# maleiwhat/Our-Tree

Hardware: AMD Instinct MI355X
Metric: GB/s AES-128-CTR (whole node) (higher is better)
Workload: dtype uint8

## Files before the change

csrc/cpu/bs_selftest.cpp:

```cpp
#include <stdio.h>
#include <stdlib.h>
#include <string.h>

#include <utility>

#include "aes.h"
#include "otc_bitslice.h"

using namespace otc_bs;


template <int... G, int... Q>
static void dfs_step(W *m, int step, std::integer_sequence<int, G...>, std::integer_sequence<int, Q...>)
{
    ((step == G ? transpose32_nib8<G>(m) : (void)0), ...);
    ((step == 8 + Q ? transpose32_quad<Q>(m) : (void)0), ...);
    ((step == 16 + G ? transpose32_group8<G>(m) : (void)0), ...);
}

extern "C" int otc_bs_dfs_transpose(uint32_t *m, const int *steps, int nsteps)
{
    for (int i = 0; i < nsteps; ++i) {
        const int s = steps[i];
        if (!((s >= 0 && s < 4) || (s >= 8 && s < 16) || (s >= 16 && s < 20))) return -1;
    }
    transpose32_bytes(m);
    for (int i = 0; i < nsteps; ++i)
        dfs_step(m, steps[i], std::make_integer_sequence<int, 4>{}, std::make_integer_sequence<int, 8>{});
    return 0;
}

extern "C" int otc_bs_ctr_out_model(const uint32_t *planes, const uint32_t *rk, const uint32_t *pt, uint32_t *out,
                                    int dfs, int ls, int first, int cap, int *order)
{
    W s[128];
    for (int p = 0; p < 128; ++p) s[p] = planes[p];
    int issued[32], emitted[32], nemit = 0, err = 0;
    uint32_t reg[32][4];
    for (int k = 0; k < 32; ++k) {
        issued[k] = k < first;
        emitted[k] = 0;
        for (int w = 0; w < 4; ++w) reg[k][w] = issued[k] ? pt[4 * k + w] : 0xDEADBEEFu;
        if (order) order[k] = -1;
    }
    auto emit = [&](int k) {
        if (!issued[k]) err = err ? err : 1;
        if (emitted[k]++) err = err ? err : 2;
        for (int w = 0; w < 4; ++w) out[4 * k + w] = x3(reg[k][w], s[32 * w + k], rk[w]);
        ++nemit;
    };
    auto issue = [&](int j) {
        if (j < first || issued[j]++) err = err ? err : 2;
        for (int w = 0; w < 4; ++w) reg[j][w] = pt[4 * j + w];
        if (order) order[j] = nemit;
    };
    if (!dfs) {
        for (int w = 0; w < 4; ++w) transpose32(s + 32 * w);
        for (int j = first; j < 32; ++j) issue(j);
        for (int k = 0; k < 32; ++k) emit(k);
    } else if (ls == 8 && first == 10 && cap == 36) {
        ctr_out_dfs<8, 10, 36>(s, emit, issue);
    } else if (ls == 8 && first == 10 && cap == 34) {
        ctr_out_dfs<8, 10, 34>(s, emit, issue);
    } else if (ls == 12 && first == 14 && cap == 36) {
        ctr_out_dfs<12, 14, 36>(s, emit, issue);
    } else if (ls == 0 && first == 4 && cap == 40) {
        ctr_out_dfs<0, 4, 40>(s, emit, issue);
    } else {
        return -1;
    }
    for (int k = 0; k < 32; ++k)
        if (!issued[k] || emitted[k] != 1) err = err ? err : 2;
    return err;
}

extern "C" int otc_bitslice_selftest(int verbose)
{
    const uint8_t *SB = aes_sbox();
    int fails = 0;
    for (int batch = 0; batch < 8; ++batch) {
        W x[8] = {0};
        for (int k = 0; k < 32; ++k) {
            int v = batch * 32 + k;
            for (int i = 0; i < 8; ++i) x[i] |= (W)((v >> i) & 1) << k;
        }
        sbox(x[0], x[1], x[2], x[3], x[4], x[5], x[6], x[7]);
        for (int k = 0; k < 32; ++k) {
            int v = batch * 32 + k, o = 0;
            for (int i = 0; i < 8; ++i) o |= (int)((x[i] >> k) & 1) << i;
            if (o != SB[v]) {
                if (verbose) printf("  sbox mismatch at %02x: %02x vs %02x\n", v, o, SB[v]);
                ++fails;
            }
        }
    }
    for (int kv = 0; kv < 256; kv += 37) {
        W k[8], x[8] = {0}, y[8];
        for (int i = 0; i < 8; ++i) k[i] = ((kv >> i) & 1) ? ~0u : 0u;
        for (int slot = 0; slot < 32; ++slot)
            for (int i = 0; i < 8; ++i) x[i] |= (W)(((slot * 7 + kv) >> i) & 1) << slot;
        for (int i = 0; i < 8; ++i) y[i] = x[i] ^ k[i];
        sbox(y[0], y[1], y[2], y[3], y[4], y[5], y[6], y[7]);
        W z[8];
        for (int i = 0; i < 8; ++i) z[i] = x[i];
        sbox_k<false>(x[0], x[1], x[2], x[3], x[4], x[5], x[6], x[7], k[0], k[1], k[2], k[3], k[4], k[5], k[6], k[7]);
        sbox_lut3(z[0], z[1], z[2], z[3], z[4], z[5], z[6], z[7], k[0], k[1], k[2], k[3], k[4], k[5], k[6], k[7]);
        for (int i = 0; i < 8; ++i)
            if (x[i] != y[i] || z[i] != y[i]) {
                if (verbose) printf("  sbox_k/sbox_lut3 mismatch kv=%d bit %d\n", kv, i);
                ++fails;
            }
    }
    for (int t = 0; t < 64; ++t) {
        W a[32], b[32];
        uint64_t z = 0x9E3779B97F4A7C15ull * (uint64_t)(t + 1);
        for (int i = 0; i < 32; ++i) {
            z ^= z << 13; z ^= z >> 7; z ^= z << 17;
            a[i] = b[i] = (W)(z >> 11);
        }
        W c[32];
        for (int i = 0; i < 32; ++i) c[i] = a[i];
        transpose32(a);
        transpose32_ref(b);
        for (int i = 0; i < 32; ++i)
            if (a[i] != b[i]) {
                if (verbose) printf("  transpose32 mismatch (trial %d, word %d)\n", t, i);
                ++fails;
                break;
// ... 81 lines not shown
                else round_step<0>(s, kr);
            }
            round_final(s, [&](int p) -> W { return kf(ctx.nr - 1, p); });
            bad = 0;
            for (int w = 0; w < 4; ++w) {
                W m[32];
                for (int q = 0; q < 32; ++q) m[q] = s[32 * w + q];
                transpose32(m);
                for (int k = 0; k < 32; ++k) {
                    uint32_t v = m[k] ^ rk[4 * ctx.nr + w];
                    bad += memcmp(&v, &ref[k][4 * w], 4) != 0;
                }
            }
            if (verbose)
                printf("  bitsliced AES-%d rolled rounds%s: %s\n", bits,
                       mixt == 2 ? " (searched 55-node MixColumns)" : mixt ? " (low-register MixColumns)" : "",
                       bad ? "failed" : "passed");
            fails += bad;
        }

        {
            static uint32_t tab[14 * 16 * OTC_BS_KT_STRIDE];
            key_term_table(rk, ctx.nr, tab);
            for (int w = 0; w < 4; ++w) {
                W m[32];
                for (int k = 0; k < 32; ++k) memcpy(&m[k], &pt[k][4 * w], 4);
                transpose32(m);
                for (int q = 0; q < 32; ++q) s[32 * w + q] = m[q];
            }
            for (int r = 0; r + 1 < ctx.nr; ++r)
                round_step_kt<true>(s, [&](int b, W *t) {
                    for (int j = 0; j < OTC_SBOX_KEY_TERMS; ++j) t[j] = tab[(r * 16 + b) * OTC_BS_KT_STRIDE + j];
                });
            round_final_kt(s, [&](int b, W *t) {
                for (int j = 0; j < OTC_SBOX_KEY_TERMS; ++j) t[j] = tab[((ctx.nr - 1) * 16 + b) * OTC_BS_KT_STRIDE + j];
            });
            bad = 0;
            for (int w = 0; w < 4; ++w) {
                W m[32];
                for (int q = 0; q < 32; ++q) m[q] = s[32 * w + q];
                transpose32(m);
                for (int k = 0; k < 32; ++k) {
                    uint32_t v = m[k] ^ rk[4 * ctx.nr + w];
                    bad += memcmp(&v, &ref[k][4 * w], 4) != 0;
                }
            }
            if (verbose) printf("  bitsliced AES-%d key-term table rounds: %s\n", bits, bad ? "failed" : "passed");
            fails += bad;

            bad = 0;
            for (int trial = 0; trial < 4; ++trial) {
                uint64_t hi = ((uint64_t)rand() << 32) ^ (uint64_t)rand();
                uint64_t lo = (((uint64_t)rand() << 32) ^ (uint64_t)rand()) & ~(uint64_t)2047u;
                if (trial == 3) lo = ~(uint64_t)0 << 11;
                const uint32_t u5 = (uint32_t)(lo >> 11) & 31u;
                uint8_t ctr[16];
                for (int b = 0; b < 8; ++b) ctr[b] = (uint8_t)(hi >> (8 * (7 - b)));
                for (int b = 0; b < 8; ++b) ctr[8 + b] = (uint8_t)(lo >> (8 * (7 - b)));
                uint8_t pre[14];
                ctr_group_prefix(lo, hi, false, 0, pre);
                bad += memcmp(pre, ctr, 14) != 0;
                static uint32_t grp[OTC_BS_CTR_GRP_WORDS];
                uint32_t c8[8], e1w[OTC_BS_CTR_E1_WORDS];
                ctr_group_consts(pre, rk, sbox_value, c8, grp);
                const uint32_t k14 = (rk[3] >> 16) & 0xFFu, k15 = rk[3] >> 24;
                ctr_e1_task(c8, k14, u5, sbox_value, e1w);
                for (int lane = 0; lane < 64; lane += 21) {
                    uint32_t ent[8];
                    ctr_e0_lane(c8, k15, (uint32_t)lane, sbox_value, ent);
                    W e0[32], e1[32];
                    for (int p = 0; p < 32; ++p) {
                        e0[p] = rep_byte(ent[p >> 2], p & 3);
                        e1[p] = e1w[p];
                    }
                    ctr_round2_mix(e0, e1, s);
                    round_step_kt<true>(s, [&](int b, W *t) {
                        for (int j = 0; j < OTC_SBOX_KEY_TERMS; ++j) t[j] = grp[b * OTC_BS_KT_STRIDE + j];
                    });
                    for (int r = 3; r + 1 < ctx.nr; ++r)
                        round_step_kt<true>(s, [&](int b, W *t) {
                            for (int j = 0; j < OTC_SBOX_KEY_TERMS; ++j) t[j] = tab[(r * 16 + b) * OTC_BS_KT_STRIDE + j];
                        });
                    round_final_kt(s, [&](int b, W *t) {
                        for (int j = 0; j < OTC_SBOX_KEY_TERMS; ++j)
                            t[j] = tab[((ctx.nr - 1) * 16 + b) * OTC_BS_KT_STRIDE + j];
                    });
                    for (int w = 0; w < 4; ++w) {
                        W m[32];
                        for (int q = 0; q < 32; ++q) m[q] = s[32 * w + q];
                        transpose32(m);
                        for (int k = 0; k < 32; ++k) {
                            uint8_t cb[16], ks[16];
                            memcpy(cb, ctr, 16);
                            const uint32_t add = 64u * (uint32_t)k + (uint32_t)lane;
                            cb[15] = (uint8_t)add;
                            cb[14] = (uint8_t)((u5 << 3) | (add >> 8));
                            aes_crypt_ecb(&ctx, AES_ENCRYPT, cb, ks);
                            uint32_t v = m[k] ^ rk[4 * ctx.nr + w];
                            bad += memcmp(&v, &ks[4 * w], 4) != 0;
                        }
                    }
                }
            }
            if (verbose) printf("  bitsliced AES-%d counter-cached CTR task: %s\n", bits, bad ? "failed" : "passed");
            fails += bad;
        }
    }
    return fails ? 1 : 0;
}
```

csrc/hip/aes_bs.hip:

```cpp
#include <hip/hip_runtime.h>

#include <cstdlib>
#include <cstring>
#include <type_traits>

#include "otc_bitslice.h"
#include "otc_device.h"
#include "otc_kernels.h"

using namespace otc_dev;
using namespace otc_bs;

namespace {

struct BsParams {
    const uint8_t *in;
    uint8_t *out;
    uint64_t nblocks;
    uint32_t tail;
    uint32_t wrap64;
    uint64_t shift;
    Ctr128 cbase;
    const uint32_t *ktab;
    const uint32_t *ctab;
// ... 73 lines not shown
        task = gw == 0 ? 0 : P.tasks - 1;
    }
    t.vbase = task * 2048u;
    if (t.vbase >= P.nblocks + shift) return false;
    t.full = t.vbase >= shift && t.vbase + 2048u - shift <= P.nblocks;
    if (P.part == BS_FULL_ONLY && !t.full) return false;
    if (P.part == BS_EDGE_ONLY && t.full) return false;
    return true;
}

#ifndef OTC_BS_NT
#define OTC_BS_NT 1
#endif
constexpr bool BS_NT = OTC_BS_NT != 0;
constexpr bool BS_NT_IN = BS_NT;
constexpr int BS_LDS_AUX = BS_NT ? 2 : 0;
__device__ __forceinline__ uint4 ld_stream(const uint8_t *p) { return ld_u4<BS_NT>(p); }
__device__ __forceinline__ void st_stream(uint8_t *p, uint4 v) { st_u4<BS_NT>(p, v); }

template <int MODE>
__device__ __forceinline__ void ecb_load_planes(const BsParams &P, const Task &t, W *s, bool full)
{
    constexpr int64_t BACK = MODE == BS_CFB_DEC ? 16 : 0;
    const uint8_t *tb = P.in + (int64_t)(t.vbase * 16) - BACK;
    const uint32_t lo = t.lane * 16u;
    uint4 blk[32];
#pragma unroll
    for (int k = 0; k < 32; ++k) {
        const uint64_t i = t.vbase + t.lane + 64u * k;
        if constexpr (MODE == BS_CFB_DEC_SEG) {
            blk[k] = seg_prev<MODE>(P, tb + lo + 1024u * k, i, full || i < P.nblocks);
        } else if (MODE == BS_CFB_DEC && k == 0) {
            const bool first = i == 0;
            const uint8_t *src = P.in + (int64_t)(t.vbase * 16) + lo - (first ? 0 : 16);
            blk[k] = blend_iv((full || i < P.nblocks) ? *(const uint4 *)src : make_uint4(0, 0, 0, 0), first, P);
        } else {
            blk[k] = (full || i < P.nblocks) ? ld_u4<BS_NT_IN>(tb + lo + 1024u * k) : make_uint4(0, 0, 0, 0);
        }
    }
#pragma unroll
    for (int w = 0; w < 4; ++w) {
        W m[32];
#pragma unroll
        for (int k = 0; k < 32; ++k) m[k] = w == 0 ? blk[k].x : w == 1 ? blk[k].y : w == 2 ? blk[k].z : blk[k].w;
        transpose32(m);
        pin_n(m, 32);
#pragma unroll
        for (int q = 0; q < 32; ++q) s[32 * w + q] = m[q];
        sched_fence();
    }
}

template <bool DEC>
__global__ __launch_bounds__(256) void k_bs_key_table(otc_aes_key K, uint32_t *tab)
{
    const int e = (int)threadIdx.x;
    if (e >= K.nr * 16) return;
    const int r = e >> 4, b = e & 15;
    uint32_t byte = (K.rk[4 * r + (b >> 2)] >> (8 * (b & 3))) & 0xFFu;
    if (DEC) byte = dec_round_key_byte(byte, r);
    W k[8];
#pragma unroll
    for (int i = 0; i < 8; ++i) k[i] = ((byte >> i) & 1u) ? ~0u : 0u;
    W t[OTC_SBOX_KEY_TERMS];
    sbox_key_terms(k[0], k[1], k[2], k[3], k[4], k[5], k[6], k[7], t);
    uint32_t *o = tab + e * OTC_BS_KT_STRIDE;
#pragma unroll
    for (int j = 0; j < OTC_SBOX_KEY_TERMS; ++j) o[j] = t[j];
    o[OTC_SBOX_KEY_TERMS] = 0;
}

using ktab_ptr = const __attribute__((address_space(4))) uint32_t *;

template <int R>
struct TableTerms {
    ktab_ptr tp;
    __device__ __forceinline__ void operator()(int b, W *t) const
    {
        ktab_ptr q = tp;
        asm volatile("" : "+s"(q));
#pragma unroll
        for (int j = 0; j < OTC_SBOX_KEY_TERMS; ++j) t[j] = q[(R * 16 + b) * OTC_BS_KT_STRIDE + j];
    }
};

template <int BASE>
struct GroupTerms {
    ktab_ptr gp;
    __device__ __forceinline__ void operator()(int b, W *t) const
    {
        ktab_ptr q = gp;
        asm volatile("" : "+s"(q));
#pragma unroll
        for (int j = 0; j < OTC_SBOX_KEY_TERMS; ++j) t[j] = q[(BASE + b) * OTC_BS_KT_STRIDE + j];
    }
};

__global__ __launch_bounds__(256) void k_bs_ctr_table(otc_aes_key K, Ctr128 cbase, uint32_t wrap64,
                                                      uint64_t ngroups, uint64_t tasks, uint32_t *gtab,
                                                      uint32_t *e0tab, uint32_t *e1tab)
{
    __shared__ uint32_t sbt[256];
    sbt[threadIdx.x] = sbox_value(threadIdx.x);
    __syncthreads();
    const auto sb = [&](uint32_t v) { return sbt[v & 0xFFu]; };
    const uint64_t i = (uint64_t)blockIdx.x * 256u + threadIdx.x;
    auto rk0b = [&](int b) -> uint32_t { return (K.rk[b >> 2] >> (8 * (b & 3))) & 0xFFu; };
    uint64_t g;
    int kind;
    if (i < ngroups) {
        g = i;
        kind = 0;
    } else if (i < ngroups * 65) {
        g = (i - ngroups) >> 6;
        kind = 1;
    } else if (i < ngroups * 65 + tasks) {
        g = (((cbase.lo >> 11) & 31u) + (i - ngroups * 65)) >> 5;
        kind = 2;
    } else {
        return;
    }
    uint8_t pre[14];
    ctr_group_prefix(cbase.lo, cbase.hi, wrap64 != 0, g, pre);
    uint32_t c8[8];
    if (kind == 0) {
        ctr_group_consts(pre, K.rk, sb, c8, gtab + g * OTC_BS_CTR_GRP_WORDS);
    } else if (kind == 1) {
        ctr_group_consts(pre, K.rk, sb, c8, (uint32_t *)nullptr);
        const uint32_t lane = (uint32_t)(i - ngroups) & 63u;
        ctr_e0_lane(c8, rk0b(15), lane, sb, e0tab + (g * 64 + lane) * 8);
    } else {
        ctr_group_consts(pre, K.rk, sb, c8, (uint32_t *)nullptr);
        const uint64_t t = i - ngroups * 65;
        const uint32_t u5 = (uint32_t)((cbase.lo >> 11) + t) & 31u;
        ctr_e1_task(c8, rk0b(14), u5, sb, e1tab + t * OTC_BS_CTR_E1_WORDS);
    }
}

template <int R, int NR, int MIX, bool DEC = false>
__device__ __forceinline__ void rounds_table(W *s, ktab_ptr tp)
{
    if constexpr (R < NR - 1) {
        round_step_kt<MIX, TableTerms<R>, 2, DEC>(s, TableTerms<R>{tp});
        pin_n(s, 128);
        rounds_table<R + 1, NR, MIX, DEC>(s, tp);
    } else {
        round_final_kt<TableTerms<NR - 1>, DEC>(s, TableTerms<NR - 1>{tp});
    }
}

#ifndef OTC_BS_CBC_D
#define OTC_BS_CBC_D 4
#endif
#ifndef OTC_BS_CFB_D
#define OTC_BS_CFB_D 2
#endif
#ifndef OTC_BS_PRE
#define OTC_BS_PRE 2
#endif
#ifndef OTC_BS_OUT_DFS
#define OTC_BS_OUT_DFS 1
#endif
#ifndef OTC_BS_DFS_CAP
#define OTC_BS_DFS_CAP 36
#endif
constexpr bool BS_OUT_DFS = OTC_BS_OUT_DFS != 0;
constexpr int BS_DFS_CAP = OTC_BS_DFS_CAP;
template <int NR, int MODE, int LS, bool CACHE, bool FO, int MIX = 2, int PRE = OTC_BS_PRE, int D = 8>
__device__ __forceinline__ void aes_bs_task(const BsParams &P, const otc_aes_key &K, uint4 *stage,
                                            int64_t claimed = -1)
{
    Task t;
    if (!task_of<MODE>(P, t, claimed)) return;
    const uint32_t lane = t.lane, wave = t.wave;
    const uint64_t shift = (MODE == BS_CTR) ? P.shift : 0;
    const bool full = FO || t.full;
    W s[128];
    auto prefetch = [&]() {
    if (MODE == BS_CTR && LS > 0) {
        const int64_t t0 = (int64_t)t.vbase - (int64_t)shift;
        const uint8_t *ib0 = P.in + t0 * 16 + lane * 16u;
#pragma unroll
        for (int k = 0; k < LS; ++k) {
            const int64_t si = t0 + (int64_t)lane + 64 * k;
            const bool ok = full || (si >= 0 && (uint64_t)si < P.nblocks);
            __builtin_amdgcn_global_load_lds((const void *)(ok ? ib0 + 1024u * k : P.in),
                                             (__attribute__((address_space(3))) void *)&stage[(wave * LS + k) * 64],
                                             16, 0, BS_LDS_AUX);
        }
    }
    };
    if (!(MODE == BS_CTR && CACHE)) prefetch();
    if (MODE == BS_CTR && CACHE) {
        const uint64_t task = t.vbase >> 11;
        const uint64_t g = (((P.cbase.lo >> 11) & 31u) + task) >> 5;
        const uint4 *q0 = (const uint4 *)(P.e0tab + (g * 64u + lane) * 8u);
        const uint4 a = q0[0], b = q0[1];
        const W ew[8] = {a.x, a.y, a.z, a.w, b.x, b.y, b.z, b.w};
        W e0[32];
#pragma unroll
        for (int p = 0; p < 32; ++p) e0[p] = rep_byte(ew[p >> 2], p & 3);
        const ktab_ptr e1p = (ktab_ptr)P.e1tab + task * OTC_BS_CTR_E1_WORDS;
        W e1[32];
#pragma unroll
        for (int p = 0; p < 32; ++p) e1[p] = e1p[p];
        const ktab_ptr gp = (ktab_ptr)P.ctab + g * OTC_BS_CTR_GRP_WORDS;
        ctr_round2_mix(e0, e1, s);
        pin_n(s, 128);
        sched_fence();
        prefetch();
        sched_fence();
        round_step_kt<MIX, GroupTerms<0>, 2>(s, GroupTerms<0>{gp});
        pin_n(s, 128);
        sched_fence();
        rounds_table<3, NR, MIX>(s, (ktab_ptr)P.ktab);
    } else if (MODE == BS_CTR) {
        const uint64_t clo = P.cbase.lo + t.vbase;
        const uint64_t chi = P.cbase.hi + ((!P.wrap64 && clo < P.cbase.lo) ? 1u : 0u);
        uint32_t cw[4] = {(uint32_t)clo, (uint32_t)(clo >> 32), (uint32_t)chi, (uint32_t)(chi >> 32)};
#pragma unroll
        for (int j = 0; j < 4; ++j) asm volatile("" : "+v"(cw[j]));
#pragma unroll
        for (int b = 0; b < 16; ++b) {
#pragma unroll
            for (int i = 0; i < 8; ++i) {
                const int n = 8 * (15 - b) + i;
                W v;
                if (n < 6) {
                    v = lane_mask(lane, n);
                } else if (n < 11) {
                    constexpr W pat[5] = {0xAAAAAAAAu, 0xCCCCCCCCu, 0xF0F0F0F0u, 0xFF00FF00u, 0xFFFF0000u};
                    v = pat[n - 6];
                } else {
                    v = (W)(0u - ((cw[n >> 5] >> (n & 31)) & 1u));
                }
                s[8 * b + i] = v;
            }
        }
#pragma unroll
        for (int q = 0; q < 128; ++q) asm volatile("" : "+v"(s[q]));
    } else {
        ecb_load_planes<MODE>(P, t, s, full);
    }
    constexpr bool DEC = MODE == BS_ECB_DEC || is_cbcd<MODE>;
    if (DEC) {
        dec_premap(s);
        pin_n(s, 128);
    }
    if (!(MODE == BS_CTR && CACHE)) {
        sched_fence();
        rounds_table<0, NR, MIX, DEC>(s, (ktab_ptr)P.ktab);
    }
    pin_n(s, 128);
    sched_fence();

// ... 60 lines not shown
            if ((k & 3) == 0) {
                sched_fence();
#pragma unroll
                for (int j = LS + PRE_; j < 32; ++j)
                    if ((j - D_ < 0 ? 0 : ((j - D_) & ~3)) == k) issue(j);
            }
            emit(k);
        }
    }
}

#ifndef OTC_BS_LS
#define OTC_BS_LS 8
#endif
constexpr int BS_LS = OTC_BS_LS;


template <int NR, int MODE, int LS, bool CACHE, bool FO>
__global__ __launch_bounds__(256) __attribute__((amdgpu_waves_per_eu(3, 3))) void k_aes_bs_t3(BsParams P,
                                                                                             otc_aes_key K)
{
    __shared__ uint4 stage[LS > 0 ? BS_WPG * LS * 64 : 1];
    aes_bs_task<NR, MODE, LS, CACHE, FO>(P, K, stage);
}

template <int NR, int MODE>
__global__ __launch_bounds__(256) __attribute__((amdgpu_waves_per_eu(3, 3))) void k_aes_bs_claim(BsParams P,
                                                                                               otc_aes_key K)
{
    strace(3);
    const uint32_t w = blockIdx.x * 4u + __builtin_amdgcn_readfirstlane(threadIdx.x >> 6);
    for (int64_t u = first_unit(P.cl, false, w); u >= 0; u = claim_unit(P.cl, false)) {
        BsParams Q = P;
        auto gin = (__attribute__((address_space(1))) const uint8_t *)P.in;
        auto gout = (__attribute__((address_space(1))) uint8_t *)P.out;
        asm volatile("" : "+s"(gin), "+s"(gout));
        Q.in = (const uint8_t *)gin;
        Q.out = (uint8_t *)gout;
        aes_bs_task<NR, MODE, 0, false, true>(Q, K, nullptr, u);
    }
}

template <int NR, int MODE>
hipError_t launch_nr(const BsParams &P, const otc_aes_key &K, hipStream_t st)
{
    const uint64_t vt = P.nblocks + (MODE == BS_CTR ? P.shift : 0);
    const uint64_t tasks = (vt + 2047) / 2048;
    uint64_t wgs = (tasks + BS_WPG - 1) / BS_WPG;
    if (wgs < 1) wgs = 1;
    if (wgs > 0xFFFFFFFFull) return hipErrorInvalidValue;
    const dim3 g((unsigned)wgs), b(64 * BS_WPG);
    bool cache = MODE == BS_CTR;
    const uint64_t ngroups = cache ? (((P.cbase.lo >> 11) & 31u) + tasks + 31) >> 5 : 0;
    const size_t ctab_words =
        cache ? ngroups * (OTC_BS_CTR_GRP_WORDS + OTC_BS_CTR_E0_WORDS) + tasks * OTC_BS_CTR_E1_WORDS : 0;
    const size_t kt_words = (size_t)NR * 16 * OTC_BS_KT_STRIDE;
    uint32_t *tab = nullptr;
    hipError_t e = hipErrorOutOfMemory;
    if (cache) {
        e = alloc_fault() ? hipErrorOutOfMemory : ws_alloc((void **)&tab, (kt_words + ctab_words) * 4, st);
        if (e != hipSuccess) {
            (void)hipGetLastError();
            cache = false;
        }
    }
    if (!cache) e = alloc_fault() ? hipErrorOutOfMemory : ws_alloc((void **)&tab, kt_words * 4, st);
    if (e != hipSuccess) return e;
    hipLaunchKernelGGL(k_bs_key_table<MODE == BS_ECB_DEC || is_cbcd<MODE>>, dim3(1), dim3(256), 0, st, K, tab);
    BsParams Q = P;
    Q.ktab = tab;
    Q.tasks = tasks;
    constexpr int LS = MODE == BS_CTR ? BS_LS : 0;
    if constexpr (MODE != BS_CTR) {
        (void)g;
        if (!P.cl.ctr) {
            (void)ws_free(tab, st);
            return hipErrorInvalidValue;
        }
        hipLaunchKernelGGL((k_aes_bs_claim<NR, MODE>),
                           dim3(P.cl.wgs ? P.cl.wgs : (unsigned)otc_dev::device_cus()), dim3(256), 0, st, Q, K);
    } else {
        const bool edge = P.shift != 0 || vt % 2048 != 0;
        auto run = [&](auto cachec) {
            constexpr bool C = decltype(cachec)::value;
            Q.part = BS_FULL_ONLY;
            hipLaunchKernelGGL((k_aes_bs_t3<NR, MODE, LS, C, true>), g, b, 0, st, Q, K);
            if (edge) {
                Q.part = BS_EDGE_ONLY;
                hipLaunchKernelGGL((k_aes_bs_t3<NR, MODE, LS, C, false>), dim3((2 + BS_WPG - 1) / BS_WPG), b, 0, st,
                                   Q, K);
            }
        };
        if (cache) {
            uint32_t *gt = tab + kt_words, *e0 = gt + ngroups * OTC_BS_CTR_GRP_WORDS,
                     *e1 = e0 + ngroups * OTC_BS_CTR_E0_WORDS;
            Q.ctab = gt;
            Q.e0tab = e0;
            Q.e1tab = e1;
            const uint64_t n = ngroups * 65 + tasks;
            hipLaunchKernelGGL(k_bs_ctr_table, dim3((unsigned)((n + 255) / 256)), dim3(256), 0, st, K, P.cbase,
                               P.wrap64, ngroups, tasks, gt, e0, e1);
        }
        if (cache)
            run(std::true_type{});
        else
            run(std::false_type{});
    }
    e = hipGetLastError();
    const hipError_t f = ws_free(tab, st);
    return e != hipSuccess ? e : f;
}

template <int MODE>
hipError_t launch(const BsParams &P, const otc_aes_key &K, hipStream_t st)
{
    return otc_impl::with_rounds(K.nr, [&](auto nr) { return launch_nr<decltype(nr)::value, MODE>(P, K, st); });
}

}

namespace otc_impl {

OTC_STRACE_READER(strace_read_bs)

hipError_t bs_ctr(const void *in, void *out, size_t nbytes, const otc_aes_key &K, Ctr128 c, bool wrap64,
                  hipStream_t st)
{
    if (nbytes % 16) {
        const size_t full = nbytes - nbytes % 16;
        Ctr128 ct = c;
        ct.lo = c.lo + full / 16;
        if (!wrap64 && ct.lo < c.lo) ct.hi += 1;
        hipError_t e = tt_ctr((const uint8_t *)in + full, (uint8_t *)out + full, nbytes % 16, K, ct, wrap64, st);
        if (e != hipSuccess) return e;
        nbytes = full;
        if (nbytes == 0) return hipSuccess;
    }
    BsParams P{};
    P.in = (const uint8_t *)in;
    P.out = (uint8_t *)out;
    P.nblocks = nbytes / 16;
    P.tail = (uint32_t)(nbytes % 16);
    P.wrap64 = wrap64 ? 1u : 0u;
    P.shift = c.lo & 2047u;
    P.cbase.lo = c.lo & ~(uint64_t)2047u;
    P.cbase.hi = c.hi;
    return launch<BS_CTR>(P, K, st);
}

hipError_t bs_preload()
{
    hipFuncAttributes a;
    return hipFuncGetAttributes(&a, reinterpret_cast<const void *>(&k_aes_bs_claim<14, BS_ECB>));
}
// ... 29 lines not shown
```

csrc/include/otc.h:

```cpp
#ifndef OTC_H
#define OTC_H

#include <stddef.h>
#include <stdint.h>

#ifdef __cplusplus
extern "C" {
#endif

#define OTC_OK 0
#define OTC_ERR_ARG -1
#define OTC_ERR_HIP -2
#define OTC_ERR_RCCL -3
#define OTC_ERR_UNSUPPORTED -4
#define OTC_ERR_NOMEM -5

const char *otc_last_error(void);

#define OTC_DIR_ENCRYPT 1
#define OTC_DIR_DECRYPT 0

typedef struct {
    uint32_t rk[60];
    int32_t nr;
// ... 196 lines not shown

int otc_device_numa_node(int dev);
int otc_engine_numa_node(const otc_engine *e);
const void *otc_engine_staging(const otc_engine *e, int slot);

#define OTC_PTR_HOST 0
#define OTC_PTR_PINNED 1
#define OTC_PTR_DEVICE 2
int otc_ptr_kind(const void *p);

int otc_host_register(void *p, size_t nbytes);
int otc_host_unregister(void *p);
void *otc_host_alloc_pinned(size_t nbytes);
void otc_host_free_pinned(void *p);

typedef struct {
    double total_ms;
    double gbps;
    int ngpus;
    int strategy;
    int numa_nodes_used;
} otc_multi_stats;

int otc_multi_run(int ngpus, int strategy, int mode, const void *host_in, void *host_out,
                  size_t nbytes, const otc_aes_key *k, const uint8_t iv_or_ctr[16], int impl,
                  size_t chunk_bytes, otc_multi_stats *stats);

typedef struct {
    uint64_t round_off;
    uint64_t round_bytes;
    uint64_t pad_bytes;
    uint64_t off, bytes;
    uint64_t blk0;
    int64_t halo;
} otc_rccl_piece;
uint64_t otc_rccl_nrounds(uint64_t nbytes, int ngpus, uint64_t piece);
int otc_rccl_plan_piece(uint64_t nbytes, int ngpus, uint64_t piece, uint64_t r, int g, otc_rccl_piece *out);
uint64_t otc_rccl_halo_start(uint64_t nbytes, uint64_t piece, uint64_t i);

void otc_multi_release(void);
void otc_release_resources(void);

void otc_fault_inject_alloc(long after);
long otc_fault_inject_pending(void);

int otc_multi_ctr_resident(int ngpus, void *const *dev_bufs, size_t shard_bytes,
                           const otc_aes_key *k, const uint8_t ctr0[16], int impl,
                           double *elapsed_ms);

int otc_bitslice_selftest(int verbose);
int otc_bs_dfs_transpose(uint32_t *m, const int *steps, int nsteps);
int otc_bs_ctr_out_model(const uint32_t *planes, const uint32_t *rk, const uint32_t *pt, uint32_t *out, int dfs,
                         int ls, int first, int cap, int *order);
const char *otc_build_info(void);
int otc_runtime_info(char *buf, size_t n);

#ifdef __cplusplus
}
#endif

#endif
```

csrc/include/otc_bitslice.h:

```cpp
#ifndef OTC_BITSLICE_H
#define OTC_BITSLICE_H

#include <stdint.h>

#if defined(__HIPCC__) || defined(__HIP__)
#define OTC_HD __host__ __device__ __forceinline__
#else
#define OTC_HD inline
#endif



namespace otc_bs {

typedef uint32_t W;

OTC_HD void sbox(W &x0, W &x1, W &x2, W &x3, W &x4, W &x5, W &x6, W &x7)
{
    const W U0 = x7, U1 = x6, U2 = x5, U3 = x4, U4 = x3, U5 = x2, U6 = x1, U7 = x0;
    const W T1 = U0 ^ U3, T2 = U0 ^ U5, T3 = U0 ^ U6, T4 = U3 ^ U5, T5 = U4 ^ U6;
    const W T6 = T1 ^ T5, T7 = U1 ^ U2, T8 = U7 ^ T6, T9 = U7 ^ T7, T10 = T6 ^ T7;
    const W T11 = U1 ^ U5, T12 = U2 ^ U5, T13 = T3 ^ T4, T14 = T6 ^ T11, T15 = T5 ^ T11;
    const W T16 = T5 ^ T12, T17 = T9 ^ T16, T18 = U3 ^ U7, T19 = T7 ^ T18, T20 = T1 ^ T19;
    const W T21 = U6 ^ U7, T22 = T7 ^ T21, T23 = T2 ^ T22, T24 = T2 ^ T10, T25 = T20 ^ T17;
// ... 354 lines not shown
        W t[8];
        lmap_byte(s + 8 * b, t);
#pragma unroll
        for (int i = 0; i < 8; ++i) s[8 * b + i] = t[i];
    }
}

OTC_HD uint32_t lmap_value(uint32_t v)
{
    uint32_t o = 0;
    for (int i = 0; i < 8; ++i)
        o |= (((v >> ((i + 2) & 7)) ^ (v >> ((i + 5) & 7)) ^ (v >> ((i + 7) & 7))) & 1u) << i;
    return o;
}
OTC_HD uint32_t dec_round_key_byte(uint32_t k, int r) { return lmap_value(k) ^ 0x05u ^ (r > 0 ? 0x63u : 0u); }

template <class KF>
struct KeyMasks {
    KF kf;
    OTC_HD void operator()(int b, W *t) const
    {
        const int p = 8 * b;
        sbox_key_terms(kf(p), kf(p + 1), kf(p + 2), kf(p + 3), kf(p + 4), kf(p + 5), kf(p + 6), kf(p + 7), t);
    }
};

template <int MIX, class KF, int FENCE = 2>
OTC_HD void round_step(W *s, KF kf)
{
    round_step_kt<MIX, KeyMasks<KF>, FENCE>(s, KeyMasks<KF>{kf});
}

template <class KF>
OTC_HD void round_final(W *s, KF kf)
{
    round_final_kt(s, KeyMasks<KF>{kf});
}

#define OTC_BS_KT_STRIDE 12
OTC_HD void key_term_table(const uint32_t *rk, int nr, uint32_t *tab)
{
    for (int r = 0; r < nr; ++r)
        for (int b = 0; b < 16; ++b) {
            const uint32_t byte = (rk[4 * r + (b >> 2)] >> (8 * (b & 3))) & 0xFFu;
            W k[8];
            for (int i = 0; i < 8; ++i) k[i] = ((byte >> i) & 1u) ? ~0u : 0u;
            uint32_t *t = tab + (r * 16 + b) * OTC_BS_KT_STRIDE;
            sbox_key_terms(k[0], k[1], k[2], k[3], k[4], k[5], k[6], k[7], t);
            t[OTC_SBOX_KEY_TERMS] = 0;
        }
}

#define OTC_BS_CTR_GRP_WORDS (16 * OTC_BS_KT_STRIDE)
#define OTC_BS_CTR_E0_WORDS (64 * 8)
#define OTC_BS_CTR_E1_WORDS 32

OTC_HD uint32_t sbox_value(uint32_t v)
{
    W x[8];
    for (int i = 0; i < 8; ++i) x[i] = (v >> i) & 1u;
    sbox(x[0], x[1], x[2], x[3], x[4], x[5], x[6], x[7]);
    uint32_t r = 0;
    for (int i = 0; i < 8; ++i) r |= (x[i] & 1u) << i;
    return r;
}
OTC_HD uint32_t xtime_value(uint32_t a) { return ((a << 1) ^ ((a & 0x80u) ? 0x1Bu : 0u)) & 0xFFu; }
OTC_HD uint32_t gmul123(uint32_t c, uint32_t a) { return c == 1 ? a : c == 2 ? xtime_value(a) : xtime_value(a) ^ a; }

OTC_HD void mix_column_bytes(const uint32_t *a, uint32_t *o)
{
    for (int r = 0; r < 4; ++r) {
        const uint32_t a0 = a[r], a1 = a[(r + 1) & 3], a2 = a[(r + 2) & 3], a3 = a[(r + 3) & 3];
        o[r] = xtime_value(a0) ^ xtime_value(a1) ^ a1 ^ a2 ^ a3;
    }
}

OTC_HD void shift_mix_bytes(const uint32_t *in, uint32_t *out)
{
    for (int c = 0; c < 4; ++c) {
        uint32_t col[4];
        for (int r = 0; r < 4; ++r) col[r] = in[r + 4 * ((c + r) & 3)];
        mix_column_bytes(col, out + 4 * c);
    }
}

OTC_HD void key_terms_of_byte(uint32_t byte, uint32_t *t)
{
    W k[8];
    for (int i = 0; i < 8; ++i) k[i] = ((byte >> i) & 1u) ? ~0u : 0u;
    sbox_key_terms(k[0], k[1], k[2], k[3], k[4], k[5], k[6], k[7], t);
    t[OTC_SBOX_KEY_TERMS] = 0;
}

OTC_HD void ctr_group_prefix(uint64_t cbase_lo, uint64_t cbase_hi, bool wrap64, uint64_t g, uint8_t *pre)
{
    const uint64_t base = cbase_lo & ~(uint64_t)0xFFFF;
    const uint64_t lo = base + (g << 16);
    const uint64_t hi = cbase_hi + ((!wrap64 && lo < base) ? 1u : 0u);
    for (int b = 0; b < 8; ++b) pre[b] = (uint8_t)(hi >> (8 * (7 - b)));
    for (int b = 0; b < 6; ++b) pre[8 + b] = (uint8_t)(lo >> (8 * (7 - b)));
}

template <class SB>
OTC_HD void ctr_group_consts(const uint8_t *pre, const uint32_t *rk, SB sb, uint32_t *c8, uint32_t *terms)
{
    auto rkb = [&](int r, int b) -> uint32_t { return (rk[4 * r + (b >> 2)] >> (8 * (b & 3))) & 0xFFu; };
    uint32_t a[16], B[16];
    for (int b = 0; b < 14; ++b) a[b] = sb(pre[b] ^ rkb(0, b));
    a[14] = a[15] = 0;
    shift_mix_bytes(a, B);
    for (int b = 0; b < 8; ++b) c8[b] = B[b] ^ rkb(1, b);
    if (terms) {
        uint32_t d[16], Q[16];
        for (int b = 0; b < 8; ++b) d[b] = 0;
        for (int b = 8; b < 16; ++b) d[b] = sb(B[b] ^ rkb(1, b));
        shift_mix_bytes(d, Q);
        for (int b = 0; b < 16; ++b) key_terms_of_byte(Q[b] ^ rkb(2, b), terms + b * OTC_BS_KT_STRIDE);
    }
}

template <class SB>
OTC_HD void ctr_e0_lane(const uint32_t *c8, uint32_t k15, uint32_t lane, SB sb, uint32_t *out)
{
    const uint32_t cf[4] = {1, 1, 3, 2};
    uint32_t e[4][4];
#pragma unroll
    for (uint32_t q = 0; q < 4; ++q) {
        const uint32_t s15 = sb((lane | (q << 6)) ^ k15);
#pragma unroll
        for (int j = 0; j < 4; ++j) e[q][j] = sb(c8[j] ^ gmul123(cf[j], s15));
    }
#pragma unroll
    for (int w = 0; w < 8; ++w) {
        uint32_t v = 0;
#pragma unroll
        for (int b = 0; b < 4; ++b) {
            const int p = 4 * w + b, j = p >> 3, i = p & 7;
            uint32_t nib = 0;
#pragma unroll
            for (int q = 0; q < 4; ++q) nib |= ((e[q][j] >> i) & 1u) << q;
            v |= (nib | (nib << 4)) << (8 * b);
        }
        out[w] = v;
    }
}

template <class SB>
OTC_HD void ctr_e1_task(const uint32_t *c8, uint32_t k14, uint32_t u5, SB sb, uint32_t *out)
{
    const uint32_t cf[4] = {1, 3, 2, 1};
    uint32_t e[8][4];
#pragma unroll
    for (uint32_t w = 0; w < 8; ++w) {
        const uint32_t s14 = sb((w | (u5 << 3)) ^ k14);
#pragma unroll
        for (int j = 0; j < 4; ++j) e[w][j] = sb(c8[4 + j] ^ gmul123(cf[j], s14));
    }
#pragma unroll
    for (int p = 0; p < 32; ++p) {
        uint32_t v = 0;
#pragma unroll
        for (uint32_t w = 0; w < 8; ++w) v |= ((e[w][p >> 3] >> (p & 7)) & 1u) * (0xFu << (4 * w));
        out[p] = v;
    }
}

OTC_HD W rep_byte(W x, int b)
{
#if defined(__HIP_DEVICE_COMPILE__)
    return __builtin_amdgcn_perm(x, x, 0x01010101u * (uint32_t)b);
#else
    return ((x >> (8 * b)) & 0xFFu) * 0x01010101u;
#endif
// ... 250 lines not shown
```

our_tree_amd/_native.py:

```python
from __future__ import annotations

import atexit
import ctypes
import os
import threading

_HERE = os.path.dirname(os.path.abspath(__file__))
LIB_DIR = os.path.join(_HERE, "lib")
GPU_LIB_PATH = os.environ.get("OTC_LIB") or os.path.join(LIB_DIR, "libotc.so")
CPU_LIB_PATH = os.path.join(LIB_DIR, "libotc_cpu.so")

_lock = threading.Lock()
_gpu_lib = None
_cpu_lib = None

c_u8p = ctypes.POINTER(ctypes.c_uint8)
c_vp = ctypes.c_void_p
c_sz = ctypes.c_size_t
c_u64 = ctypes.c_uint64
c_int = ctypes.c_int


class OtcAesKey(ctypes.Structure):

# ... 88 lines not shown

def _declare_cpu(lib):
    P = ctypes.POINTER
    sig = {
        "aes_setkey_enc": (c_int, [P(AesContext), c_u8p, ctypes.c_uint]),
        "aes_setkey_dec": (c_int, [P(AesContext), c_u8p, ctypes.c_uint]),
        "aes_crypt_ecb": (c_int, [P(AesContext), c_int, c_u8p, c_u8p]),
        "aes_crypt_cbc": (c_int, [P(AesContext), c_int, c_sz, c_u8p, c_u8p, c_u8p]),
        "aes_crypt_cfb128": (c_int, [P(AesContext), c_int, c_sz, P(c_int), c_u8p, c_u8p, c_u8p]),
        "aes_crypt_ctr": (c_int, [P(AesContext), c_int, P(c_int), c_u8p, c_u8p, c_u8p, c_u8p]),
        "aes_self_test": (c_int, [c_int]),
        "aes_export_rk32": (c_int, [P(AesContext), P(ctypes.c_uint32)]),
        "aes_ctr_bulk": (c_int, [P(AesContext), c_u8p, c_u8p, c_u8p, c_sz, c_int]),
        "aes_ecb_bulk": (c_int, [P(AesContext), c_int, c_u8p, c_u8p, c_sz, c_int]),
        "aes_ctr128_add": (None, [c_u8p, c_u64]),
        "aes_xts_setkey_enc": (c_int, [P(AesXtsContext), c_u8p, ctypes.c_uint]),
        "aes_xts_setkey_dec": (c_int, [P(AesXtsContext), c_u8p, ctypes.c_uint]),
        "aes_crypt_xts": (c_int, [P(AesXtsContext), c_int, c_sz, c_u8p, c_u8p, c_u8p]),
        "aes_crypt_xts_units": (c_int, [P(AesXtsContext), c_int, c_sz, c_sz, c_u8p, c_u8p, c_u8p]),
        "aes_gcm_setkey": (c_int, [P(AesGcmContext), c_u8p, ctypes.c_uint]),
        "aes_gcm_set_h": (None, [P(AesGcmContext), c_u8p]),
        "aes_gf128_mul": (None, [c_u8p, c_u8p, c_u8p]),
        "aes_ghash": (None, [P(AesGcmContext), c_u8p, c_u8p, c_sz]),
        "aes_gcm_j0": (None, [P(AesGcmContext), c_u8p, c_sz, c_u8p]),
        "aes_crypt_ctr32": (c_int, [P(AesGcmContext), c_sz, c_u8p, c_u8p, c_u8p]),
        "aes_crypt_gcm": (c_int, [P(AesGcmContext), c_int, c_sz, c_u8p, c_sz, c_u8p, c_sz, c_u8p, c_u8p, c_u8p]),
        "aes_gcm_auth_decrypt": (c_int, [P(AesGcmContext), c_sz, c_u8p, c_sz, c_u8p, c_sz, c_u8p, c_sz, c_u8p, c_u8p]),
        "chacha20_block": (None, [c_u8p, c_u8p, ctypes.c_uint32, c_u8p]),
        "chacha20_crypt": (c_int, [c_u8p, c_u8p, ctypes.c_uint32, c_u8p, c_u8p, c_sz]),
        "poly1305_mac": (None, [c_u8p, c_u8p, c_sz, c_u8p]),
        "chacha20_poly1305_encrypt": (c_int, [c_u8p, c_u8p, c_u8p, c_sz, c_u8p, c_u8p, c_sz, c_u8p]),
        "chacha20_poly1305_auth_decrypt": (c_int, [c_u8p, c_u8p, c_u8p, c_sz, c_u8p, c_u8p, c_u8p, c_sz]),
        "chacha20_poly1305_tag": (c_int, [c_u8p, c_u8p, c_u8p, c_sz, c_u8p, c_sz, c_u8p]),
        "arc4_setup": (None, [P(Arc4Context), c_u8p, ctypes.c_uint]),
        "arc4_prep": (c_int, [P(Arc4Context), c_sz, c_u8p]),
        "arc4_crypt": (c_int, [c_sz, c_u8p, c_u8p, c_u8p]),
        "arc4_crypt_mt": (c_int, [c_sz, c_u8p, c_u8p, c_u8p, c_int]),
        "arc4_self_test": (c_int, [c_int]),
        "rc4_init": (None, [P(Rc4State), ctypes.c_char_p, c_int]),
        "rc4_crypt": (None, [P(Rc4State), ctypes.c_char_p, ctypes.c_char_p, c_int]),
        "CheckAESSupport": (c_int, []),
        "AES_128_Key_Expansion": (None, [c_u8p, c_u8p]),
        "AES_192_Key_Expansion": (None, [c_u8p, c_u8p]),
        "AES_256_Key_Expansion": (None, [c_u8p, c_u8p]),
        "AES_Key_Expansion_Dec": (None, [c_u8p, c_u8p, c_int]),
        "AES_ECB_encrypt": (None, [c_u8p, c_u8p, ctypes.c_ulong, c_u8p, c_int]),
        "AES_ECB_decrypt": (None, [c_u8p, c_u8p, ctypes.c_ulong, c_u8p, c_int]),
        "AES_CTR_encrypt": (None, [c_u8p, c_u8p, c_u8p, c_u8p, ctypes.c_ulong, c_u8p, c_int]),
        "AES_CTR_encrypt_at": (None, [c_u8p, c_u8p, c_u8p, c_u8p, ctypes.c_ulong, c_u8p, c_int, ctypes.c_ulonglong]),
        "otc_bitslice_selftest": (c_int, [c_int]),
        "otc_bs_dfs_transpose": (c_int, [P(ctypes.c_uint32), P(c_int), c_int]),
        "otc_bs_ctr_out_model": (c_int, [P(ctypes.c_uint32), P(ctypes.c_uint32), P(ctypes.c_uint32),
                                         P(ctypes.c_uint32), c_int, c_int, c_int, c_int, P(c_int)]),
        "otc_rccl_nrounds": (c_u64, [c_u64, c_int, c_u64]),
        "otc_rccl_plan_piece": (c_int, [c_u64, c_int, c_u64, c_u64, c_int, P(RcclPiece)]),
        "otc_rccl_halo_start": (c_u64, [c_u64, c_u64, c_u64]),
        "AES_CBC_encrypt": (None, [c_u8p, c_u8p, c_u8p, ctypes.c_ulong, c_u8p, c_int]),
        "AES_CFB128_encrypt": (None, [c_u8p, c_u8p, c_u8p, ctypes.c_ulong, c_u8p, c_int]),
        "aes_monte_carlo": (c_int, [c_int, c_int, c_u8p]),
        "aes_monte_carlo_expected": (ctypes.c_char_p, [c_int, c_int]),
        "otc_parse_cpulist": (c_int, [ctypes.c_char_p, c_u8p, c_int]),
        "otc_numa_node_of_pci": (c_int, [ctypes.c_char_p, ctypes.c_char_p]),
        "otc_numa_node_cpus": (c_int, [ctypes.c_char_p, c_int, c_u8p, c_int]),
        "otc_numa_num_nodes": (c_int, [ctypes.c_char_p]),
        "otc_numa_bind_thread": (c_int, [c_int]),
        "otc_numa_alloc": (c_vp, [c_sz, c_int]),
        "otc_numa_free": (None, [c_vp, c_sz]),
        "otc_numa_node_of_addr": (c_int, [c_vp]),
    }
    for name, (res, args) in sig.items():
        fn = getattr(lib, name)
        fn.restype = res
        fn.argtypes = args


def _declare_gpu(lib):
    _declare_cpu(lib)
    P = ctypes.POINTER
    K = P(OtcAesKey)
    sig = {
        "otc_last_error": (ctypes.c_char_p, []),
        "otc_pick_impl": (c_int, [c_int, c_int, c_int, c_u64]),
        "otc_last_impl": (c_int, []),
        "otc_xts_key_init": (c_int, [P(OtcXtsKey), c_u8p, c_int, c_int]),
        "otc_aes_xts": (c_int, [c_vp, c_vp, c_sz, c_sz, P(OtcXtsKey), c_u8p, c_vp]),
        "otc_gcm_key_init": (c_int, [P(OtcGcmKey), c_u8p, c_int]),
        "otc_aes_ctr32": (c_int, [c_vp, c_vp, c_sz, K, c_u8p, c_int, c_vp]),
        "otc_ghash": (c_int, [c_vp, c_sz, c_u8p, c_u8p, c_vp, c_vp]),
        "otc_aes_gcm": (c_int, [c_vp, c_vp, c_sz, P(OtcGcmKey), c_int, c_u8p, c_sz, c_u8p, c_sz, c_vp, c_int, c_vp]),
        "otc_ghash_spans": (c_int, [P(c_u64), c_int]),
        "otc_gcm_batch_spans": (c_int, [P(c_u64), c_int]),
        "otc_gcm_batch_table_bytes": (c_sz, []),
        "otc_gcm_batch_ws_bytes": (c_sz, [c_sz]),
        "otc_gcm_batch_tables": (c_int, [P(OtcGcmKey), c_vp, c_vp]),
        "otc_gcm_batch_plan": (ctypes.c_int64, [c_vp, c_sz, c_int, c_vp, c_vp, c_vp]),
        "otc_gcm_batch_lanes": (c_int, [c_vp, c_sz]),
        "otc_ghash_batch": (c_int, [c_vp, c_sz, c_vp, c_vp, c_int, c_vp]),
        "otc_aes_gcm_batch": (c_int, [c_vp, c_vp, c_vp, c_vp, c_u64, c_int, c_sz, P(OtcGcmKey), c_vp, c_vp, c_int,
                                      c_vp, c_vp, c_vp, c_int, c_vp, c_vp, c_int, c_vp]),
        "otc_chacha20": (c_int, [c_vp, c_vp, c_sz, c_u8p, c_u8p, ctypes.c_uint32, c_vp]),
        "otc_poly1305": (c_int, [c_vp, c_sz, c_u8p, c_vp, c_vp]),
        "otc_poly1305_spans": (c_int, [P(c_u64), c_int]),
        "otc_chacha20_poly1305": (c_int, [c_vp, c_vp, c_sz, c_u8p, c_int, c_u8p, c_u8p, c_sz, c_vp, c_vp]),
        "otc_split_stats": (None, [c_int]),
        "otc_split_fallback_reason": (ctypes.c_char_p, []),
        "otc_split_last_units": (c_int, [ctypes.POINTER(c_u64), ctypes.POINTER(c_u64), ctypes.POINTER(c_u64)]),
# ... 143 lines not shown
```

Measured before the change: 1732.

## Share CTR e0/e1 tables per counter variant and fuse key-table build

The e0 and e1 counter-cache tables are now built once per counter variant, meaning each span of 2^24 groups sharing the high counter bytes, instead of per group and per task. The main kernel indexes them by variant and u5. This shrinks the setup work and the table footprint from scaling with the input size to a handful of entries, which should make those tables cache-resident. The bitsliced key-table build is folded into the CTR table kernel, saving one launch, and new host checks are added to confirm variant tables match the per-group computation.

```diff
diff --git a/csrc/cpu/bs_selftest.cpp b/csrc/cpu/bs_selftest.cpp
--- a/csrc/cpu/bs_selftest.cpp
+++ b/csrc/cpu/bs_selftest.cpp
@@ -74,6 +74,59 @@
     return err;
 }
 
+
+extern "C" uint64_t otc_bs_ctr_variant_of(uint64_t cbase_lo, uint64_t g, uint64_t *first)
+{
+    const uint64_t v = ctr_group_variant(cbase_lo, g);
+    if (first) *first = ctr_variant_first_group(cbase_lo, v);
+    return v;
+}
+
+extern "C" int otc_bs_ctr_tables_check(const uint32_t *rk, uint64_t cbase_lo, uint64_t cbase_hi, int wrap64,
+                                       uint64_t ngroups, uint64_t *nvar, uint64_t *distinct)
+{
+    if (!rk || !nvar || ngroups < 1 || ngroups > (1u << 20)) return -1;
+    uint32_t sbt[256];
+    for (uint32_t v = 0; v < 256; ++v) sbt[v] = sbox_value(v);
+    const auto sb = [&](uint32_t v) { return sbt[v & 0xFFu]; };
+    const uint32_t k14 = (rk[3] >> 16) & 0xFFu, k15 = rk[3] >> 24;
+    struct Tab {
+        uint32_t e0[OTC_BS_CTR_E0_WORDS], e1[OTC_BS_CTR_E1_WORDS];
+    };
+    static_assert(OTC_BS_CTR_E0_WORDS == 64 * 8 && OTC_BS_CTR_E1_WORDS == 32 * OTC_BS_CTR_E1_ENTRY, "table layout");
+    *nvar = ctr_group_variant(cbase_lo, ngroups - 1) + 1;
+    if (distinct) *distinct = 0;
+    Tab cur{}, prev{};
+    uint64_t have = ~(uint64_t)0;
+    int bad = 0;
+    for (uint64_t g = 0; g < ngroups; ++g) {
+        const uint64_t v = ctr_group_variant(cbase_lo, g);
+        if (v >= *nvar || (have != ~(uint64_t)0 && v != have && v != have + 1)) return -1;
+        if (v != have) {
+            prev = cur;
+            uint32_t c8[8];
+            ctr_variant_c8(cbase_lo, cbase_hi, wrap64 != 0, v, rk, sb, c8);
+            for (uint32_t lane = 0; lane < 64; ++lane) ctr_e0_lane(c8, k15, lane, sb, cur.e0 + lane * 8);
+            for (uint32_t u5 = 0; u5 < 32; ++u5) ctr_e1_task(c8, k14, u5, sb, cur.e1 + u5 * OTC_BS_CTR_E1_ENTRY);
+            if (distinct && v > 0 && memcmp(&prev, &cur, sizeof cur) != 0) ++*distinct;
+            have = v;
+        }
+        uint8_t pre[14];
+        ctr_group_prefix(cbase_lo, cbase_hi, wrap64 != 0, g, pre);
+        uint32_t c8[8], ent[OTC_BS_CTR_E1_ENTRY];
+        ctr_group_consts(pre, rk, sb, c8, (uint32_t *)nullptr);
+        for (uint32_t lane = 0; lane < 64; ++lane) {
+            ctr_e0_lane(c8, k15, lane, sb, ent);
+            bad += memcmp(ent, cur.e0 + lane * 8, 8 * sizeof(uint32_t)) != 0;
+        }
+        for (uint32_t u5 = 0; u5 < 32; ++u5) {
+            ctr_e1_task(c8, k14, u5, sb, ent);
+            bad += memcmp(ent, cur.e1 + u5 * OTC_BS_CTR_E1_ENTRY, sizeof ent) != 0;
+        }
+    }
+    return bad;
+}
+
 extern "C" int otc_bitslice_selftest(int verbose)
 {
     const uint8_t *SB = aes_sbox();
@@ -261,6 +314,7 @@
             for (int trial = 0; trial < 4; ++trial) {
                 uint64_t hi = ((uint64_t)rand() << 32) ^ (uint64_t)rand();
                 uint64_t lo = (((uint64_t)rand() << 32) ^ (uint64_t)rand()) & ~(uint64_t)2047u;
+                if (trial == 2) lo = (lo & ~(((uint64_t)1 << 40) - 1)) | (lo & 0x1F800u) | 0x10000u;
                 if (trial == 3) lo = ~(uint64_t)0 << 11;
                 const uint32_t u5 = (uint32_t)(lo >> 11) & 31u;
                 uint8_t ctr[16];
@@ -270,8 +324,11 @@
                 ctr_group_prefix(lo, hi, false, 0, pre);
                 bad += memcmp(pre, ctr, 14) != 0;
                 static uint32_t grp[OTC_BS_CTR_GRP_WORDS];
-                uint32_t c8[8], e1w[OTC_BS_CTR_E1_WORDS];
+                uint32_t c8[8], e1w[OTC_BS_CTR_E1_ENTRY];
                 ctr_group_consts(pre, rk, sbox_value, c8, grp);
+                const uint64_t cb = lo - ((uint64_t)3 << 16), var = ctr_group_variant(cb, 3);
+                bad += var != (trial == 2 ? 1u : 0u);
+                ctr_variant_c8(cb, hi, false, var, rk, sbox_value, c8);
                 const uint32_t k14 = (rk[3] >> 16) & 0xFFu, k15 = rk[3] >> 24;
                 ctr_e1_task(c8, k14, u5, sbox_value, e1w);
                 for (int lane = 0; lane < 64; lane += 21) {
@@ -313,6 +370,19 @@
             }
             if (verbose) printf("  bitsliced AES-%d counter-cached CTR task: %s\n", bits, bad ? "failed" : "passed");
             fails += bad;
+
+            bad = 0;
+            for (int trial = 0; trial < 6; ++trial) {
+                const uint64_t r = ((uint64_t)rand() << 32) ^ (uint64_t)rand();
+                const uint64_t hi = trial == 5 ? ~(uint64_t)0 : r * 0x9E3779B97F4A7C15ull;
+                const uint64_t top = trial < 2 ? (r | 1) << 40 : 0;
+                const uint64_t lo = top - ((uint64_t)2 << 16) - (r & 0xF800u);
+                uint64_t nvar = 0, distinct = 0;
+                const int rc = otc_bs_ctr_tables_check(rk, lo, hi, trial & 1, 6, &nvar, &distinct);
+                bad += rc != 0 || nvar != 2 || distinct != 1;
+            }
+            if (verbose) printf("  bitsliced AES-%d per-variant CTR tables: %s\n", bits, bad ? "failed" : "passed");
+            fails += bad;
         }
     }
     return fails ? 1 : 0;
diff --git a/csrc/hip/aes_bs.hip b/csrc/hip/aes_bs.hip
--- a/csrc/hip/aes_bs.hip
+++ b/csrc/hip/aes_bs.hip
@@ -149,9 +149,8 @@
 }
 
 template <bool DEC>
-__global__ __launch_bounds__(256) void k_bs_key_table(otc_aes_key K, uint32_t *tab)
-{
-    const int e = (int)threadIdx.x;
+__device__ __forceinline__ void key_table_entry(const otc_aes_key &K, int e, uint32_t *tab)
+{
     if (e >= K.nr * 16) return;
     const int r = e >> 4, b = e & 15;
     uint32_t byte = (K.rk[4 * r + (b >> 2)] >> (8 * (b & 3))) & 0xFFu;
@@ -165,6 +164,12 @@
 #pragma unroll
     for (int j = 0; j < OTC_SBOX_KEY_TERMS; ++j) o[j] = t[j];
     o[OTC_SBOX_KEY_TERMS] = 0;
+}
+
+template <bool DEC>
+__global__ __launch_bounds__(256) void k_bs_key_table(otc_aes_key K, uint32_t *tab)
+{
+    key_table_entry<DEC>(K, (int)threadIdx.x , tab);
 }
 
 using ktab_ptr = const __attribute__((address_space(4))) uint32_t *;
@@ -194,44 +199,38 @@
 };
 
 __global__ __launch_bounds__(256) void k_bs_ctr_table(otc_aes_key K, Ctr128 cbase, uint32_t wrap64,
-                                                      uint64_t ngroups, uint64_t tasks, uint32_t *gtab,
-                                                      uint32_t *e0tab, uint32_t *e1tab)
+                                                      uint64_t ngroups, uint32_t nvar, uint32_t *ktab,
+                                                      uint32_t *gtab, uint32_t *e0tab, uint32_t *e1tab)
 {
     __shared__ uint32_t sbt[256];
     sbt[threadIdx.x] = sbox_value(threadIdx.x);
     __syncthreads();
     const auto sb = [&](uint32_t v) { return sbt[v & 0xFFu]; };
-    const uint64_t i = (uint64_t)blockIdx.x * 256u + threadIdx.x;
+    uint64_t i = (uint64_t)blockIdx.x * 256u + threadIdx.x;
     auto rk0b = [&](int b) -> uint32_t { return (K.rk[b >> 2] >> (8 * (b & 3))) & 0xFFu; };
-    uint64_t g;
-    int kind;
+    uint32_t c8[8];
     if (i < ngroups) {
-        g = i;
-        kind = 0;
-    } else if (i < ngroups * 65) {
-        g = (i - ngroups) >> 6;
-        kind = 1;
-    } else if (i < ngroups * 65 + tasks) {
-        g = (((cbase.lo >> 11) & 31u) + (i - ngroups * 65)) >> 5;
-        kind = 2;
-    } else {
+        uint8_t pre[14];
+        ctr_group_prefix(cbase.lo, cbase.hi, wrap64 != 0, i, pre);
+        ctr_group_consts(pre, K.rk, sb, c8, gtab + i * OTC_BS_CTR_GRP_WORDS);
         return;
     }
-    uint8_t pre[14];
-    ctr_group_prefix(cbase.lo, cbase.hi, wrap64 != 0, g, pre);
-    uint32_t c8[8];
-    if (kind == 0) {
-        ctr_group_consts(pre, K.rk, sb, c8, gtab + g * OTC_BS_CTR_GRP_WORDS);
-    } else if (kind == 1) {
-        ctr_group_consts(pre, K.rk, sb, c8, (uint32_t *)nullptr);
-        const uint32_t lane = (uint32_t)(i - ngroups) & 63u;
-        ctr_e0_lane(c8, rk0b(15), lane, sb, e0tab + (g * 64 + lane) * 8);
-    } else {
-        ctr_group_consts(pre, K.rk, sb, c8, (uint32_t *)nullptr);
-        const uint64_t t = i - ngroups * 65;
-        const uint32_t u5 = (uint32_t)((cbase.lo >> 11) + t) & 31u;
-        ctr_e1_task(c8, rk0b(14), u5, sb, e1tab + t * OTC_BS_CTR_E1_WORDS);
-    }
+    i -= ngroups;
+    if (i < (uint64_t)nvar * 64u) {
+        const uint32_t lane = (uint32_t)i & 63u;
+        ctr_variant_c8(cbase.lo, cbase.hi, wrap64 != 0, i >> 6, K.rk, sb, c8);
+        ctr_e0_lane(c8, rk0b(15), lane, sb, e0tab + i * 8u);
+        return;
+    }
+    i -= (uint64_t)nvar * 64u;
+    if (i < (uint64_t)nvar * 32u) {
+        const uint32_t u5 = (uint32_t)i & 31u;
+        ctr_variant_c8(cbase.lo, cbase.hi, wrap64 != 0, i >> 5, K.rk, sb, c8);
+        ctr_e1_task(c8, rk0b(14), u5, sb, e1tab + i * OTC_BS_CTR_E1_ENTRY);
+        return;
+    }
+    i -= (uint64_t)nvar * 32u;
+    if (i < 256) key_table_entry<false>(K, (int)i, ktab);
 }
 
 template <int R, int NR, int MIX, bool DEC = false>
@@ -291,13 +290,15 @@
     if (MODE == BS_CTR && CACHE) {
         const uint64_t task = t.vbase >> 11;
         const uint64_t g = (((P.cbase.lo >> 11) & 31u) + task) >> 5;
-        const uint4 *q0 = (const uint4 *)(P.e0tab + (g * 64u + lane) * 8u);
+        const uint64_t v = ctr_group_variant(P.cbase.lo, g);
+        const uint32_t u5 = (uint32_t)((P.cbase.lo >> 11) + task) & 31u;
+        const uint4 *q0 = (const uint4 *)(P.e0tab + (v * 64u + lane) * 8u);
         const uint4 a = q0[0], b = q0[1];
         const W ew[8] = {a.x, a.y, a.z, a.w, b.x, b.y, b.z, b.w};
         W e0[32];
 #pragma unroll
         for (int p = 0; p < 32; ++p) e0[p] = rep_byte(ew[p >> 2], p & 3);
-        const ktab_ptr e1p = (ktab_ptr)P.e1tab + task * OTC_BS_CTR_E1_WORDS;
+        const ktab_ptr e1p = (ktab_ptr)P.e1tab + (v * 32u + u5) * OTC_BS_CTR_E1_ENTRY;
         W e1[32];
 #pragma unroll
         for (int p = 0; p < 32; ++p) e1[p] = e1p[p];
@@ -464,8 +465,9 @@
     const dim3 g((unsigned)wgs), b(64 * BS_WPG);
     bool cache = MODE == BS_CTR;
     const uint64_t ngroups = cache ? (((P.cbase.lo >> 11) & 31u) + tasks + 31) >> 5 : 0;
+    const uint64_t nvar = cache ? ctr_group_variant(P.cbase.lo, ngroups - 1) + 1 : 0;
     const size_t ctab_words =
-        cache ? ngroups * (OTC_BS_CTR_GRP_WORDS + OTC_BS_CTR_E0_WORDS) + tasks * OTC_BS_CTR_E1_WORDS : 0;
+        cache ? ngroups * OTC_BS_CTR_GRP_WORDS + nvar * (OTC_BS_CTR_E0_WORDS + OTC_BS_CTR_E1_WORDS) : 0;
     const size_t kt_words = (size_t)NR * 16 * OTC_BS_KT_STRIDE;
     uint32_t *tab = nullptr;
     hipError_t e = hipErrorOutOfMemory;
@@ -478,7 +480,8 @@
     }
     if (!cache) e = alloc_fault() ? hipErrorOutOfMemory : ws_alloc((void **)&tab, kt_words * 4, st);
     if (e != hipSuccess) return e;
-    hipLaunchKernelGGL(k_bs_key_table<MODE == BS_ECB_DEC || is_cbcd<MODE>>, dim3(1), dim3(256), 0, st, K, tab);
+    if (!cache)
+        hipLaunchKernelGGL(k_bs_key_table<MODE == BS_ECB_DEC || is_cbcd<MODE>>, dim3(1), dim3(256), 0, st, K, tab);
     BsParams Q = P;
     Q.ktab = tab;
     Q.tasks = tasks;
@@ -505,13 +508,13 @@
         };
         if (cache) {
             uint32_t *gt = tab + kt_words, *e0 = gt + ngroups * OTC_BS_CTR_GRP_WORDS,
-                     *e1 = e0 + ngroups * OTC_BS_CTR_E0_WORDS;
+                     *e1 = e0 + nvar * OTC_BS_CTR_E0_WORDS;
             Q.ctab = gt;
             Q.e0tab = e0;
             Q.e1tab = e1;
-            const uint64_t n = ngroups * 65 + tasks;
+            const uint64_t n = ngroups + nvar * (64 + 32) + NR * 16;
             hipLaunchKernelGGL(k_bs_ctr_table, dim3((unsigned)((n + 255) / 256)), dim3(256), 0, st, K, P.cbase,
-                               P.wrap64, ngroups, tasks, gt, e0, e1);
+                               P.wrap64, ngroups, (uint32_t)nvar, tab, gt, e0, e1);
         }
         if (cache)
             run(std::true_type{});
diff --git a/csrc/include/otc.h b/csrc/include/otc.h
--- a/csrc/include/otc.h
+++ b/csrc/include/otc.h
@@ -272,6 +272,9 @@
 int otc_bs_dfs_transpose(uint32_t *m, const int *steps, int nsteps);
 int otc_bs_ctr_out_model(const uint32_t *planes, const uint32_t *rk, const uint32_t *pt, uint32_t *out, int dfs,
                          int ls, int first, int cap, int *order);
+int otc_bs_ctr_tables_check(const uint32_t *rk, uint64_t cbase_lo, uint64_t cbase_hi, int wrap64, uint64_t ngroups,
+                            uint64_t *nvar, uint64_t *distinct);
+uint64_t otc_bs_ctr_variant_of(uint64_t cbase_lo, uint64_t g, uint64_t *first);
 const char *otc_build_info(void);
 int otc_runtime_info(char *buf, size_t n);
 
diff --git a/csrc/include/otc_bitslice.h b/csrc/include/otc_bitslice.h
--- a/csrc/include/otc_bitslice.h
+++ b/csrc/include/otc_bitslice.h
@@ -430,8 +430,9 @@
 }
 
 #define OTC_BS_CTR_GRP_WORDS (16 * OTC_BS_KT_STRIDE)
+#define OTC_BS_CTR_E1_ENTRY 32
 #define OTC_BS_CTR_E0_WORDS (64 * 8)
-#define OTC_BS_CTR_E1_WORDS 32
+#define OTC_BS_CTR_E1_WORDS (32 * OTC_BS_CTR_E1_ENTRY)
 
 OTC_HD uint32_t sbox_value(uint32_t v)
 {
@@ -497,6 +498,20 @@
     }
 }
 
+OTC_HD uint64_t ctr_group_variant(uint64_t cbase_lo, uint64_t g) { return (((cbase_lo >> 16) + g) >> 24) - (cbase_lo >> 40); }
+OTC_HD uint64_t ctr_variant_first_group(uint64_t cbase_lo, uint64_t v)
+{
+    return v ? (((cbase_lo >> 40) + v) << 24) - (cbase_lo >> 16) : 0;
+}
+template <class SB>
+OTC_HD void ctr_variant_c8(uint64_t cbase_lo, uint64_t cbase_hi, bool wrap64, uint64_t v, const uint32_t *rk, SB sb,
+                           uint32_t *c8)
+{
+    uint8_t pre[14];
+    ctr_group_prefix(cbase_lo, cbase_hi, wrap64, ctr_variant_first_group(cbase_lo, v), pre);
+    ctr_group_consts(pre, rk, sb, c8, (uint32_t *)nullptr);
+}
+
 template <class SB>
 OTC_HD void ctr_e0_lane(const uint32_t *c8, uint32_t k15, uint32_t lane, SB sb, uint32_t *out)
 {
diff --git a/our_tree_amd/_native.py b/our_tree_amd/_native.py
--- a/our_tree_amd/_native.py
+++ b/our_tree_amd/_native.py
@@ -164,6 +164,8 @@
         "otc_bs_dfs_transpose": (c_int, [P(ctypes.c_uint32), P(c_int), c_int]),
         "otc_bs_ctr_out_model": (c_int, [P(ctypes.c_uint32), P(ctypes.c_uint32), P(ctypes.c_uint32),
                                          P(ctypes.c_uint32), c_int, c_int, c_int, c_int, P(c_int)]),
+        "otc_bs_ctr_tables_check": (c_int, [P(ctypes.c_uint32), c_u64, c_u64, c_int, c_u64, P(c_u64), P(c_u64)]),
+        "otc_bs_ctr_variant_of": (c_u64, [c_u64, c_u64, P(c_u64)]),
         "otc_rccl_nrounds": (c_u64, [c_u64, c_int, c_u64]),
         "otc_rccl_plan_piece": (c_int, [c_u64, c_int, c_u64, c_u64, c_int, P(RcclPiece)]),
         "otc_rccl_halo_start": (c_u64, [c_u64, c_u64, c_u64]),
```

Result: no change. 1744 (median of 6 runs) (+0.7%).
